# Jisu-Linnea-Han/ClimateMachine.jl

Hardware: AMD Instinct MI355X
Metric: DG RHS DOF-updates/sec (higher is better)
Workload: dtype f64; 1 GPU; Held-Suarez dry GCM (BASELINE configs[2]), stacked cubed sphere 6x30x30x8 elements, N=4, LSRK54 explicit, hyperdiffusion (DryBiharmonic, horizontal), Rusanov, fp64; elements=43200, nodes_per_element=125, states=5, parallelism=element partition (Hilbert, whole columns), 1 rank(s), RCCL p2p halo

## Files before the change

climatemachine.jl_amd/_lib.py:

```python
import ctypes as C
import os

_HERE = os.path.dirname(os.path.abspath(__file__))
LIB_PATH = os.environ.get("CMDG_LIB", os.path.join(_HERE, "libcmdg.so"))

CMDG_K = dict(GRADIENTS=0, DIVGRAD=1, GRADLAP=2, TENDENCY=3, PACK=4, UNPACK=5, UPDATE_AUX=6,
              FILTER=7, STACK_INTEGRAL=8, TRANSPORT=9, HALO_EXPOSED=10, GRADIENTS_EXT=11,
              DIVGRAD_EXT=12, GRADLAP_EXT=13, TENDENCY_EXT=14, FV_GRADIENTS=15, FV_TENDENCY=16,
              ESDG_TENDENCY=17)
STACK_MAXOUT = 8
OPT_KEEP_GRADFLUX = 1
OPT_STACK_HEIGHT = 2
OPT_REFERENCE_HALO = 3
OPT_HALO_PIPELINE = 4
OPT_STEP_GRAPH = 5
OPT_STREAM_PRIORITY = 6
OPT_TENDENCY_PAIRS = 7
OPT_ASYNC_RUN = 8
OPT_TENDENCY_FOUR_WAVES = 9
OPT_GRADARG_HANDOFF = 10
CMDG_Q = dict(GRADFLUX_LIVE=1, LAW_NEEDS_GRADFLUX=2, NDERIVED=3, NUPDATED_AUX=4, FUSED_UPDATE_AUX=5,
              DIRECT_SEND=6, DIRECT_RECV=7, TENDENCY_ELEMS_PER_GROUP=8, HALO_PIPELINE=9, HOST_POST_NS=10, HOST_POST_COUNT=11, GRAPH_STEPS=12, TENDENCY_PAIRS=13,
              GRADARG_HANDOFF=14, GRADARG_REFRESHES=15,
              STATE_READ=16, AUX_READ=20)
# ... 107 lines not shown
    _fields_ = [("volume_flux", C.c_int32), ("surface_flux", C.c_int32), ("Mcut", C.c_double),
                ("low_mach", C.c_int32), ("kinetic_energy_preserving", C.c_int32)]


(ESDG_FLUX_NONE, ESDG_FLUX_ENTROPY_CONSERVATIVE, ESDG_FLUX_CENTRAL, ESDG_FLUX_KG, ESDG_FLUX_RUSANOV,
 ESDG_FLUX_ENTROPY_CONSERVATIVE_PENALTY, ESDG_FLUX_MATRIX) = range(7)
FV_VANLEER, FV_NOLIMITER = 0, 1


_vp, _i32, _i64, _d = C.c_void_p, C.c_int32, C.c_int64, C.c_double
SYMBOLS = [
    ("cmdg_version", C.c_char_p, []),
    ("cmdg_status_string", C.c_char_p, [C.c_int]),
    ("cmdg_physics_counts", C.c_int, [_i32, _vp, _vp]),
    ("cmdg_atmos_host_constants", C.c_int, [_vp, _vp, _vp]),
    ("cmdg_create", C.c_int, [C.POINTER(CmdgDesc), C.POINTER(_vp)]),
    ("cmdg_create_dgfv", C.c_int, [C.POINTER(CmdgDesc), C.POINTER(CmdgFvDesc), C.POINTER(_vp)]),
    ("cmdg_create_esdg", C.c_int, [C.POINTER(CmdgDesc), C.POINTER(CmdgEsdgDesc), C.POINTER(_vp)]),
    ("cmdg_esdg_entropy", C.c_int, [_vp, _vp, _vp, _vp]),
    ("cmdg_destroy", C.c_int, [_vp]),
    ("cmdg_last_error", C.c_char_p, [_vp]),
    ("cmdg_rhs", C.c_int, [_vp, _vp, _vp, _d, _d, _d]),
    ("cmdg_rhs_async", C.c_int, [_vp, _vp, _vp, _d, _d, _d]),
    ("cmdg_lsrk_step", C.c_int, [_vp, _vp, _vp, _d, _d, _i32, _vp, _vp, _vp]),
    ("cmdg_lsrk_run", C.c_int, [_vp, _vp, _vp, _d, _d, _i64, _i32, _vp, _vp, _vp]),
    ("cmdg_synchronize", C.c_int, [_vp]),
    ("cmdg_set_option", C.c_int, [_vp, _i32, _i32]),
    ("cmdg_query", C.c_int, [_vp, _i32, _vp]),
    ("cmdg_export_hypervisc_grad", C.c_int, [_vp, _vp]),
    ("cmdg_export_gradient_flux", C.c_int, [_vp, _vp]),
# ... 108 lines not shown
```

climatemachine.jl_amd/csrc/create.hip:

```cpp
#include <dlfcn.h>

#include <algorithm>
#include <new>

#include "engine_base.h"
#include "laws.h"
#include "reductions.h"

using namespace cmdg;

static thread_local std::string g_create_err;
void cmdg::set_create_err(const std::string &msg) { g_create_err = msg; }

namespace {
struct Law {
    int32_t id;
    EngineBase *(*make)(const cmdg_desc *, std::string &);
    int (*counts)(const int32_t *iparam, int32_t out[6]);
};
const Law LAWS[] = {
    {CMDG_PHYSICS_ADVECTION_DIFFUSION, make_engine_advdiff, counts_advdiff},
    {CMDG_PHYSICS_DRY_ATMOS, make_engine_atmos, counts_atmos},
    {CMDG_PHYSICS_HYDROSTATIC_BOUSSINESQ, make_engine_ocean, counts_ocean},
    {CMDG_PHYSICS_PRESSURE_GRADIENT, make_engine_pgrad, counts_pgrad},
// ... 84 lines not shown
    if (r) g_create_err = err;
    return r;
}

int cmdg_physics_counts(int32_t physics_id, const int32_t *iparam, int32_t out[6])
{
    if (!iparam || !out) return CMDG_ERR_INVALID;
    const Law *law = find_law(physics_id);
    return law ? law->counts(iparam, out) : CMDG_ERR_UNSUPPORTED;
}

int cmdg_atmos_host_constants(const int32_t *iparam, const double *dparam, double out[7])
{
    if (!iparam || !dparam || !out) return CMDG_ERR_INVALID;
    return host_constants_atmos(iparam, dparam, out);
}

static int create_handle(const cmdg_desc *d, const cmdg_fv_desc *fv, cmdg_handle *out, const cmdg_esdg_desc *esdg = nullptr)
{
    *out = nullptr;
    int ndev = 0;
    if (hipGetDeviceCount(&ndev) != hipSuccess || ndev == 0) {
        g_create_err = "no HIP device visible";
        return CMDG_ERR_NO_DEVICE;
    }
    if (d->dim != 3 || d->N[0] != d->N[1]) {
        g_create_err = "only dim == 3 with one horizontal polynomial order is compiled in";
        return CMDG_ERR_UNSUPPORTED;
    }
    if (d->nf_first < CMDG_RUSANOV || d->nf_first > CMDG_ROE_MOIST_LVPP) {
// ... 190 lines not shown
```

climatemachine.jl_amd/csrc/engine.h:

```cpp
#pragma once
#include "engine_base.h"
#include "kernels.h"

namespace cmdg {

template <class P, int NQ_, int NQV_ = NQ_>
struct EngineT : EngineBase {
    typename P::Params prm;
    PassArgs<P> make_args(const RhsCtx &c, const int64_t *elems, int64_t n, int dir, bool exterior, double *send0,
                          double *send1) const
    {
        PassArgs<P> a;
        a.prm = prm;
        a.g = g;
        a.elems = elems;
        a.nelems = n;
        a.Q = c.Qin;
        a.aux = aux;
        a.aux_rw = aux;
        a.derived = derived;
        a.gf = gf;
        a.hypgrad = hypgrad;
        a.hypdiv = hypdiv;
        a.tendency = c.tendency;
// ... 114 lines not shown
        return CMDG_OK;
    }
    bool has_update_aux() const override { return P::HAS_UPDATE_AUX && P::update_aux_active(prm); }
    bool law_needs_gradflux() const override { return P::needs_gradflux(prm); }
    bool gf_node_major() const override { return cmdg::gf_node_major<P>::value; }
    bool fused_update_aux() const override { return P::HAS_UPDATE_AUX && P::FUSE_UPDATE_AUX; }
    bool garg_capable() const override { return HO && !P::needs_gradflux(prm); }
    bool refresh_elidable() const override { return ELIDE; }
    int law_nder() const override { return P::HAS_SOURCE ? P::NDER : 0; }
    int law_nupd() const override { return P::HAS_UPDATE_AUX ? P::NUPD : 0; }
    int tendency_epb() const override { return TendencyShape<P, NQ_, NQV_>::EPB; }
    int law_state_read(int pass) const override { return law_reads<P>::state(pass); }
    int law_aux_read(int pass) const override { return law_reads<P>::aux(pass); }
    int init_derived() override
    {
        if constexpr (P::NDER > 0) {
            const int64_t n = nelem * KDims<NQ_, NQV_>::Np;
            if (derived.alloc((size_t)n * P::NDER) != hipSuccess)
                return fail(CMDG_ERR_HIP, "hipMalloc(derived) failed");
            hipLaunchKernelGGL((k_init_derived<P, NQ_, NQV_>), dim3((unsigned)((n + 255) / 256)), dim3(256),
                               0, s_comp, prm, aux, derived, nelem);
            if (hipStreamSynchronize(s_comp) != hipSuccess)
                return fail(CMDG_ERR_HIP, "k_init_derived failed");
        }
        return CMDG_OK;
    }
};

template <class P, int NQ_, int NQV_ = NQ_>
EngineBase *make_engine(const cmdg_desc *d)
// ... 17 lines not shown
```

climatemachine.jl_amd/csrc/engine_atmos.hip:

```cpp
#include "engine.h"
#include "laws.h"
#include "physics_atmos.h"
#include "with_constant.h"

namespace cmdg {

int counts_atmos(const int32_t *ip, int32_t out[6])
{
    const bool orient = ip[0] != 0, ref = ip[1] != 0, hyp = ip[4] != 0, smag = ip[14] == 1;
    out[0] = 5;
    out[1] = 3 + (orient ? 4 : 0) + (ref ? 7 : 0) + (smag ? 1 : 0) + (hyp ? 1 : 0) + 2;
    out[2] = 4 + (smag ? 1 : 0) + (hyp ? 4 : 0);
    out[3] = 9 + (smag ? 1 : 0);
    out[4] = hyp ? 4 : 0;
    out[5] = hyp ? 12 : 0;
    return CMDG_OK;
}

int host_constants_atmos(const int32_t *ip, const double *dp, double out[7])
{
    static_assert(ATMOS_NHOSTCONST == 7, "cmdg_atmos_host_constants documents seven");
    using P = DryAtmos<false, false, false>;
    P::Params prm;
    P::make_params(prm, ip, dp);
    P::host_constants(prm, out);
    return CMDG_OK;
}

template <int NQ>
static EngineBase *pick(const cmdg_desc *d, std::string &err)
{
    const bool orient = d->iparam[0] != 0, ref = d->iparam[1] != 0, hyp = d->iparam[4] != 0;
    bool mms = (d->iparam[5] & 8) != 0;
    for (int i = 0; i < d->iparam[6] && i < 7; ++i) mms = mms || d->iparam[7 + i] == 2;
    if (mms && (orient || ref || hyp || d->iparam[14] != 0)) {
        err = "DryAtmos: MMSSource / InitStateBC are compiled for NoOrientation, NoReferenceState, "
              "constant viscosity only";
        return nullptr;
    }
    if (d->nf_first >= NF_ROE) {
        if constexpr (NQ == 5) {
// ... 48 lines not shown
```

climatemachine.jl_amd/csrc/kernels.h:

```cpp
#pragma once
#include <type_traits>

#include "cmdg_common.h"

#ifndef CMDG_TEND_MINW
#define CMDG_TEND_MINW 1
#endif
#ifndef CMDG_TEND_EPB_LARGE
#define CMDG_TEND_EPB_LARGE 2
#endif
#ifndef CMDG_TEND_EPB_SMALL
#define CMDG_TEND_EPB_SMALL 1
#endif
#ifndef CMDG_GRAD_MINW
#define CMDG_GRAD_MINW 4
#endif
#ifndef CMDG_GRAD_BOUND_LARGE
#define CMDG_GRAD_BOUND_LARGE 1024
#endif
#ifndef CMDG_LAP_MINW
#define CMDG_LAP_MINW 1
#endif

namespace cmdg {
// ... 69 lines not shown
template <int NQ, int NQV = NQ>
__device__ __forceinline__ void face_setup(const GridDev &g, int64_t e, int t, int f, int n,
                                           FacePt &fp)
{
    int32_t idP;
    int bctag;
    face_index<NQ, NQV>(g, e, t, f, idP, bctag);
    face_geometry<NQ, NQV>(g, e, t, f, n, idP, bctag, fp);
}

template <class P, class = void>
struct has_flux_wavespeed : std::false_type {
};
template <class P>
struct has_flux_wavespeed<P, std::void_t<decltype(P::HAS_FLUX_WAVESPEED)>> : std::true_type {
};

template <class P, class = void>
struct gf_node_major : std::false_type {
};
template <class P>
struct gf_node_major<P, std::void_t<decltype(P::GF_NODE_MAJOR)>>
    : std::integral_constant<bool, P::GF_NODE_MAJOR && (P::NGF > 0)> {
};
template <class P, int Np>
__device__ __forceinline__ int64_t gf_at(int n, int s, int64_t e)
{
    return col_at<gf_node_major<P>::value, P::NGF, Np>(n, s, e);
}
template <class P, int Np>
// ... 254 lines not shown
        const int sidx = surf_index<NQ, NQV>(tid);
#pragma unroll
        for (int s = 0; s < NS; ++s) sQ[s * Np + tid] = lQ[s];
        if (STAGE_M && sidx >= 0) {
#pragma unroll
            for (int s = 0; s < NFA; ++s) sM[s * NSURF + sidx] = laux[P::face_aux(s)];
            if (use_gf) {
#pragma unroll
                for (int s = 0; s < NGF; ++s) sM[(NFA + s) * NSURF + sidx] = lgf[s];
            }
#pragma unroll
            for (int s = 0; s < NHYP; ++s) sM[(NFA + NGFS + s) * NSURF + sidx] = lhyp[s];
        }
        Vec<3 * NS> F, F2;
        F.negzero();
        if constexpr (NCA > 0) {
            Vec<NCA> lc;
            P::node_cache(a.prm, lc, lQ, laux);
            P::flux_first_order_cached(a.prm, F, lQ, laux, lc);
            if (sidx >= 0) {
#pragma unroll
                for (int s = 0; s < NCA; ++s)
                    sM[(OCA + s) * NSURF + sidx] = lc[s];
            }
        } else {
            P::flux_first_order(a.prm, F, lQ, laux, a_t, a.model_dir);
        }
        F2.negzero();
        P::flux_second_order(a.prm, F2, lQ, lgf, lhyp, laux, a_t);
#pragma unroll
        for (int q = 0; q < 3 * NS; ++q) F[q] += F2[q];
        if (hz) {
            if constexpr (!METRICS_FIRST) {
                x11 = vg[XI1X1 * Np], x12 = vg[XI1X2 * Np], x13 = vg[XI1X3 * Np];
                x21 = vg[XI2X1 * Np], x22 = vg[XI2X2 * Np], x23 = vg[XI2X3 * Np];
            }
#pragma unroll
            for (int s = 0; s < NS; ++s) {
                const double F1 = F[3 * s], F2_ = F[3 * s + 1], F3 = F[3 * s + 2];
// ... 1 lines not shown
                sF[(1 * NS + s) * Np + tid] = M * (x21 * F1 + x22 * F2_ + x23 * F3);
            }
        }
        if (vt) {
            if constexpr (!METRICS_FIRST) x31 = vg[XI3X1 * Np], x32 = vg[XI3X2 * Np], x33 = vg[XI3X3 * Np];
#pragma unroll
            for (int s = 0; s < NS; ++s) {
                const double F1 = F[3 * s], F2_ = F[3 * s + 1], F3 = F[3 * s + 2];
                sF[(2 * NS + s) * Np + tid] = M * (x31 * F1 + x32 * F2_ + x33 * F3);
            }
        }
        S.negzero();
        if constexpr (P::HAS_SOURCE) {
            Vec<P::NDER> lder;
            load_state<P::NDER, Np>(lder, a.derived, tid, e);
            P::source(a.prm, S, lQ, lgf, laux, lder, a_t, a.model_dir);
        }
    }
    __syncthreads();
    Vec<NS> Tv;
    if (live && tid < Np) {
        const int i = tid % NQ, j = (tid / NQ) % NQ, k = tid / (NQ * NQ);
        Vec<NS> Tprev;
#pragma unroll
        for (int s = 0; s < NS; ++s) Tprev[s] = 0.0;
        if (a.beta != 0) {
#pragma unroll
            for (int s = 0; s < NS; ++s) Tprev[s] = a.tendency[tid + (int64_t)Np * (s + (int64_t)NS * e)];
        }
        double mDi[NQ], mDj[NQ], mDk[NQV];
#pragma unroll
// ... 786 lines not shown
```

climatemachine.jl_amd/csrc/laws.h:

```cpp
#pragma once
#include <string>

#include "engine_base.h"

namespace cmdg {

EngineBase *make_engine_advdiff(const cmdg_desc *d, std::string &err);
EngineBase *make_engine_advdiff_fv(const cmdg_desc *d, const cmdg_fv_desc *fv, std::string &err);
EngineBase *make_engine_atmos(const cmdg_desc *d, std::string &err);
EngineBase *make_engine_ocean(const cmdg_desc *d, std::string &err);
EngineBase *make_engine_pgrad(const cmdg_desc *d, std::string &err);
EngineBase *make_engine_sw(const cmdg_desc *d, std::string &err);
EngineBase *make_engine_moist(const cmdg_desc *d, std::string &err);
EngineBase *make_engine_se01(const cmdg_desc *d, std::string &err);
EngineBase *make_engine_atmos_linear(const cmdg_desc *d, std::string &err);
EngineBase *make_engine_moist_linear(const cmdg_desc *d, std::string &err);
EngineBase *make_engine_atmos_acoustic(const cmdg_desc *d, std::string &err);
EngineBase *make_engine_esdg(const cmdg_desc *d, const cmdg_esdg_desc *ed, std::string &err);

int counts_advdiff(const int32_t *iparam, int32_t out[6]);
int counts_atmos(const int32_t *iparam, int32_t out[6]);
int counts_ocean(const int32_t *iparam, int32_t out[6]);
int counts_pgrad(const int32_t *iparam, int32_t out[6]);
int counts_sw(const int32_t *iparam, int32_t out[6]);
int counts_moist(const int32_t *iparam, int32_t out[6]);
int counts_ocean_se01(const int32_t *iparam, int32_t out[6]);
int counts_continuity3d_se01(const int32_t *iparam, int32_t out[6]);
int counts_barotropic_se01(const int32_t *iparam, int32_t out[6]);
int counts_atmos_linear(const int32_t *iparam, int32_t out[6]);
int counts_moist_linear(const int32_t *iparam, int32_t out[6]);
int counts_atmos_acoustic(const int32_t *iparam, int32_t out[6]);
int counts_esdg_dryatmos(const int32_t *iparam, int32_t out[6]);
int host_constants_atmos(const int32_t *iparam, const double *dparam, double out[7]);

}
```

climatemachine.jl_amd/csrc/physics_atmos.h:

```cpp
#pragma once
#include "cmdg_common.h"

namespace cmdg {

struct AtmosParams {
    int orient, subtract, kinematic, src, nbc;
    int bc[8];
    double visc, tau, R_d, cp_d, cv_d, T_0, grav, Omega, MSLP, day, invPr, C_smag;
    int withdiv, zero_h;
    double k_a, k_f, k_s;
    double kappa;
    double gamma, gamma_R;
    double R_ratio;
};
static constexpr int ATMOS_NHOSTCONST = 7;

template <bool ORIENT, bool REF, bool HYPER, bool SMAG = false, bool LAWNF = false>
struct DryAtmos {
    static constexpr bool LAW_NF = LAWNF;
    static_assert(!(SMAG && HYPER), "gradient-variable order of this combination is not laid out");
    static_assert(!SMAG || ORIENT, "SmagorinskyLilly needs an orientation (buoyancy correction)");
    using Params = AtmosParams;
    static constexpr int NS = 5;
    static constexpr int OPHI = 3;
    static constexpr int OREF = OPHI + (ORIENT ? 4 : 0);
    static constexpr int OTURB = OREF + (REF ? 7 : 0);
    static constexpr int ODELTA = OTURB + (SMAG ? 1 : 0);
    static constexpr int OMOIST = ODELTA + (HYPER ? 1 : 0);
    static constexpr int NAUX = OMOIST + 2;
    static constexpr int NGRAD = 4 + (SMAG ? 1 : 0) + (HYPER ? 4 : 0);
// ... 50 lines not shown
        p.C_smag = dp[13];
        p.withdiv = ip[15] & 1;
        p.zero_h = (ip[15] >> 1) & 1;
        derive_params(p);
    }
    static void derive_params(Params &p)
    {
        const double day = p.day, R_d = p.R_d, cp_d = p.cp_d, cv_d = p.cv_d;
        p.k_a = 1 / (40 * day);
        p.k_f = 1 / day;
        p.k_s = 1 / (4 * day);
        p.kappa = R_d / cp_d;
        p.gamma = cp_d / cv_d;
        p.gamma_R = p.gamma * R_d;
        p.R_ratio = R_d / R_d;
    }
    static void host_constants(const Params &p, double *out)
    {
        const double c[ATMOS_NHOSTCONST] = {p.k_a, p.k_f, p.k_s, p.kappa, p.gamma, p.gamma_R, p.R_ratio};
        for (int i = 0; i < ATMOS_NHOSTCONST; ++i) out[i] = c[i];
    }

    __device__ static double internal_energy(const Params &, const double *Q, const double *aux)
    {
        const double rho = Q[0];
        const double rhoinv = 1 / rho;
        const double rhoe_kin = rhoinv * (Q[1] * Q[1] + Q[2] * Q[2] + Q[3] * Q[3]) / 2;
        const double e_pot = ORIENT ? aux[OPHI] : -0.0;
        const double rhoe_pot = rho * e_pot;
        const double rhoe_int = Q[4] - rhoe_kin - rhoe_pot;
        return rhoinv * rhoe_int;
    }
    __device__ static double air_T(const Params &m, double e_int) { return m.T_0 + e_int / m.cv_d; }
    __device__ static double air_p(const Params &m, double T, double rho) { return m.R_d * rho * T; }
    __device__ static double soundspeed(const Params &m, double T)
    {
        return sqrt(m.gamma_R * T);
    }

    static constexpr bool MMS_VARIANT = !ORIENT && !REF && !HYPER && !SMAG && !LAWNF;
    static constexpr bool HAS_COURANT = true;
    static constexpr bool HAS_PENALTY = false;
    __device__ static void update_penalty(const Params &, double *, const double *, const double *,
                                          const double *)
    {
    }
    __device__ static double courant(const Params &m, int kind, const double *Q, const double *aux,
                                     const double *gf, double dx, double dt, double, int direction)
// ... 22 lines not shown
            }
            return dt * normnu / (dx * dx);
        }
        const double dotk = Q[1] * k[0] + Q[2] * k[1] + Q[3] * k[2];
        double normu;
        if (direction == DIR_VERTICAL) {
            normu = fabs(dotk) / Q[0];
        } else {
            double v[3];
#pragma unroll
            for (int d = 0; d < 3; ++d)
                v[d] = direction == DIR_HORIZONTAL ? (Q[1 + d] - dotk * k[d]) / Q[0] : Q[1 + d] / Q[0];
            normu = sqrt(v[0] * v[0] + v[1] * v[1] + v[2] * v[2]);
        }
        if (kind == 0) return dt * normu / dx;
        const double ss = soundspeed(m, air_T(m, internal_energy(m, Q, aux)));
        return dt * (normu + ss) / dx;
    }

    __device__ static void flux_first_order(const Params &m, double *F, const double *Q,
                                            const double *aux, double, int)
    {
        const double rho = Q[0];
        const double T = air_T(m, internal_energy(m, Q, aux));
        const double p = air_p(m, T, rho);
        double u[3];
#pragma unroll
        for (int d = 0; d < 3; ++d) u[d] = Q[1 + d] / rho;
#pragma unroll
        for (int d = 0; d < 3; ++d) F[d] = Q[1 + d];
        double pp = p;
        if constexpr (REF) pp = m.subtract ? p - aux[OREF + 1] : p;
#pragma unroll
        for (int c = 0; c < 3; ++c)
#pragma unroll
            for (int d = 0; d < 3; ++d)
                F[d + 3 * (1 + c)] = Q[1 + d] * u[c] + (0.0 + (d == c ? pp : 0.0));
#pragma unroll
        for (int d = 0; d < 3; ++d) F[d + 12] = u[d] * Q[4] + u[d] * p;
    }
    __device__ static double sym(const double *c, int i, int j)
    {
        const int lo = i < j ? i : j, hi = i < j ? j : i;
// ... 72 lines not shown
        }
    }
    __device__ static void init_derived(const Params &, double *der, const double *aux)
    {
        if constexpr (ORIENT) {
            const double phi =
                asin(aux[2] / sqrt(aux[0] * aux[0] + aux[1] * aux[1] + aux[2] * aux[2]));
            der[0] = sin(phi);
            der[1] = cos(phi);
        }
    }
    __device__ static void hs_coeffs(const Params &m, const double *Q, const double *der,
                                     double T, double &k_v, double &k_T, double &T_equil)
    {
        const double k_a = m.k_a, k_f = m.k_f, k_s = m.k_s;
        const double dTy = 60, dthz = 10, T_eq = 315, T_min = 200, sig_b = 7.0 / 10;
        const double p = air_p(m, T, Q[0]);
        const double sig = p / m.MSLP;
        const double exner = pow(sig, m.kappa);
        const double dsig = (sig - sig_b) / (1 - sig_b);
        const double hf = dsig > 0 ? dsig : 0;
        const double s = der[0], c = der[1];
        double Te = (T_eq - dTy * (s * s) - dthz * log(sig) * (c * c)) * exner;
        Te = Te > T_min ? Te : T_min;
        T_equil = Te;
        k_T = k_a + (k_s - k_a) * hf * ((c * c) * (c * c));
        k_v = k_f * hf;
    }
    __device__ static void source(const Params &m, double *S, const double *Q, const double *,
                                  const double *aux, const double *der, double t, int)
    {
        const double rho = Q[0];
        double Sm[3] = {0, 0, 0}, Se = 0;
        bool first = true;
        double T = 0, k_v = 0, k_T = 0, Te = 0;
        if (m.src & 4) {
            T = air_T(m, internal_energy(m, Q, aux));
            hs_coeffs(m, Q, der, T, k_v, k_T, Te);
        }
        if constexpr (ORIENT) {
            if (m.src & 1) {
                double r = rho;
                if constexpr (REF) r = m.subtract ? rho - aux[OREF] : rho;
#pragma unroll
                for (int d = 0; d < 3; ++d) Sm[d] = -r * aux[OPHI + 1 + d];
                first = false;
            }
        }
        if (m.src & 2) {
            const double w = 2 * m.Omega;
            const double c[3] = {-(0 * Q[3] - w * Q[2]), -(w * Q[1] - 0 * Q[3]),
                                 -(0 * Q[2] - 0 * Q[1])};
#pragma unroll
            for (int d = 0; d < 3; ++d) Sm[d] = first ? c[d] : Sm[d] + c[d];
            first = false;
        }
        if constexpr (ORIENT) {
            if (m.src & 4) {
                double k[3];
#pragma unroll
                for (int d = 0; d < 3; ++d) k[d] = aux[OPHI + 1 + d] / m.grav;
                const double kn = k[0] * Q[1] + k[1] * Q[2] + k[2] * Q[3];
#pragma unroll
                for (int d = 0; d < 3; ++d) {
                    const double x = -k_v * (Q[1 + d] - k[d] * kn);
                    Sm[d] = first ? x : Sm[d] + x;
                }
                first = false;
                Se = -k_T * rho * m.cv_d * (T - Te);
            }
        }
        S[0] = 0;
        S[1] = Sm[0];
        S[2] = Sm[1];
        S[3] = Sm[2];
        S[4] = Se;
// ... 88 lines not shown
    }
    __device__ static void gradient_argument(const Params &m, double *G, const double *Q,
                                             const double *aux, double)
    {
        const double rhoinv = 1 / Q[0];
#pragma unroll
        for (int d = 0; d < 3; ++d) G[d] = rhoinv * Q[1 + d];
        const double T = air_T(m, internal_energy(m, Q, aux));
        const double e_tot = Q[4] * (1 / Q[0]);
        G[3] = m.zero_h ? 0.0 : e_tot + m.R_d * T;
        if constexpr (SMAG) G[4] = theta_v(m, T, Q[0]);
        if constexpr (HYPER && ORIENT) {
            double u[3], k[3];
#pragma unroll
            for (int d = 0; d < 3; ++d) u[d] = Q[1 + d] * rhoinv;
#pragma unroll
            for (int d = 0; d < 3; ++d) k[d] = aux[OPHI + 1 + d] / m.grav;
#pragma unroll
            for (int i = 0; i < 3; ++i) {
                double acc = 0;
#pragma unroll
                for (int j = 0; j < 3; ++j) {
                    const double Pij = (i == j ? 1.0 : 0.0) - k[i] * k[j];
                    acc = j == 0 ? Pij * u[j] : acc + Pij * u[j];
                }
                G[4 + i] = acc;
            }
            G[7] = G[3];
        }
    }
    __device__ static double theta_v(const Params &m, double T, double rho)
    {
        const double exner = pow(air_p(m, T, rho) / m.MSLP, m.kappa);
        return m.R_ratio * (T / exner);
    }
    __device__ static void gradient_flux(const Params &m, double *gf, const double *g,
                                         const double *Q, const double *aux, double t)
    {
        double th = 0;
        if constexpr (SMAG) th = theta_v(m, air_T(m, internal_energy(m, Q, aux)), Q[0]);
        gradient_flux_th(m, gf, g, aux, th);
    }
    __device__ static void gradient_flux_g(const Params &m, double *gf, const double *g,
                                           const double *, const double *aux, double,
                                           const double *G)
    {
        gradient_flux_th(m, gf, g, aux, SMAG ? G[SMAG ? 4 : 0] : 0.0);
    }
    __device__ static void gradient_flux_th(const Params &, double *gf, const double *g,
                                            const double *aux, double th)
    {
        if constexpr (SMAG) {
            gf[9] = (g[0 + 3 * 4] * aux[OPHI + 1] + g[1 + 3 * 4] * aux[OPHI + 2] +
                     g[2 + 3 * 4] * aux[OPHI + 3]) / th;
        }
// ... 5 lines not shown
        gf[6] = g[1 + 3 * 1];
        gf[7] = (g[2 + 3 * 1] + g[1 + 3 * 2]) / 2;
        gf[8] = g[2 + 3 * 2];
    }
    __device__ static void post_gradient_laplacian(const Params &m, double *hyp, const double *gl,
                                                   const double *, const double *aux, double)
    {
        if constexpr (HYPER) {
            const double h = aux[ODELTA] / 2;
            const double nu4 = (h * h) * (h * h) / 2 / m.tau;
#pragma unroll
            for (int q = 0; q < 12; ++q) hyp[q] = nu4 * gl[q];
        }
    }
    __device__ static void wavespeed(const Params &m, double *ws, const double *n, const double *Q,
                                     const double *aux, double, int)
    {
        const double rhoinv = 1 / Q[0];
        const double uN =
            fabs(n[0] * (rhoinv * Q[1]) + n[1] * (rhoinv * Q[2]) + n[2] * (rhoinv * Q[3]));
        const double ss = soundspeed(m, air_T(m, internal_energy(m, Q, aux)));
#pragma unroll
        for (int s = 0; s < 5; ++s) ws[s] = uN + ss;
    }
    __device__ static double roe_average(double sM, double sP, double vM, double vP)
    {
        return (sM * vM + sP * vP) / (sM + sP);
    }
    __device__ static void numerical_flux_law(const Params &m, int nf, double *fluxn,
                                              const double *n, const double *QM,
                                              const double *auxM, const double *QP,
                                              const double *auxP, double t, int facedir)
    {
        double FM[15], FP[15];
#pragma unroll
        for (int i = 0; i < 15; ++i) FM[i] = FP[i] = -0.0;
        flux_first_order(m, FM, QM, auxM, t, facedir);
        flux_first_order(m, FP, QP, auxP, t, facedir);
        const double rM = QM[0], rP = QP[0];
        double uM[3], uP[3];
#pragma unroll
        for (int d = 0; d < 3; ++d) {
            uM[d] = QM[1 + d] / rM;
            uP[d] = QP[1 + d] / rP;
        }
        const double TM = air_T(m, internal_energy(m, QM, auxM));
        const double TP = air_T(m, internal_energy(m, QP, auxP));
        const double pM = air_p(m, TM, rM), pP = air_p(m, TP, rP);
        const double cM = soundspeed(m, TM), cP = soundspeed(m, TP);
        const double unM = uM[0] * n[0] + uM[1] * n[1] + uM[2] * n[2];
        const double unP = uP[0] * n[0] + uP[1] * n[1] + uP[2] * n[2];
        if (nf == NF_LMARS) {
            double ppM = pM, ppP = pP;
            if constexpr (REF)
                if (m.subtract) {
                    ppM -= auxM[OREF + 1];
                    ppP -= auxP[OREF + 1];
                }
            const double hM = m.zero_h ? 0.0 : QM[4] / rM + m.R_d * TM;
            const double hP = m.zero_h ? 0.0 : QP[4] / rP + m.R_d * TP;
            const double beta = 1.0;
            const double u_half = 1.0 / 2 * (unP + unM) - beta * 1 / (rM + rP) / cM * (ppP - ppM);
// ... 70 lines not shown
        } else if (0 <= SP) {
#pragma unroll
            for (int s = 0; s < 5; ++s)
                fluxn[s] += (S0 * (SP * QP[s] - fnP[s]) + SP * pD[s]) / (SP - S0);
        } else {
#pragma unroll
            for (int s = 0; s < 5; ++s) fluxn[s] += fnP[s];
        }
    }
    __device__ static void update_aux(const Params &m, const double *Q, double *aux, double)
    {
        static_assert(!GRADARG_REFRESH_UNREAD ||
                          (upd_aux(0) == NAUX - NUPD && aux_read(0) <= NAUX - NUPD &&
                           aux_read(2) <= NAUX - NUPD && aux_read(3) <= NAUX - NUPD),
                      "a pass that reads moisture.theta_v / air_T needs the refresh in every update");
        const double T = air_T(m, internal_energy(m, Q, aux));
        aux[OMOIST] = theta_v(m, T, Q[0]);
        aux[OMOIST + 1] = T;
    }
    __device__ static void boundary_state(const Params &m, int kind, int bctag, double *QP,
                                          double *auxP, const double *n, const double *QM,
                                          const double *, double t, const double *, const double *)
    {
        if constexpr (MMS_VARIANT) {
            if (m.bc[bctag - 1] == 2) {
                mms_state(t, auxP[0], auxP[1], auxP[2], QP);
                return;
            }
        }
        if (m.bc[bctag - 1] == 1) {
            const double dn = QM[1] * n[0] + QM[2] * n[1] + QM[3] * n[2];
// ... 39 lines not shown
```

include/cmdg.h:

```cpp
#ifndef CMDG_H
#define CMDG_H
#include <stdint.h>

#ifdef __cplusplus
extern "C" {
#endif

typedef struct cmdg_context *cmdg_handle;

typedef enum cmdg_status {
    CMDG_OK = 0,
    CMDG_ERR_INVALID = -1,
    CMDG_ERR_HIP = -2,
    CMDG_ERR_NO_DEVICE = -3,
    CMDG_ERR_COMM = -4,
    CMDG_ERR_UNSUPPORTED = -5
} cmdg_status;

enum { CMDG_EVERY_DIRECTION = 0, CMDG_HORIZONTAL_DIRECTION = 1, CMDG_VERTICAL_DIRECTION = 2 };
enum {
    CMDG_RUSANOV = 0, CMDG_CENTRAL_FIRST_ORDER = 1,
    CMDG_ROE = 2, CMDG_HLLC = 3, CMDG_LMARS = 4,
    CMDG_ROE_MOIST = 5, CMDG_ROE_MOIST_LM = 6, CMDG_ROE_MOIST_HH = 7, CMDG_ROE_MOIST_LV = 8,
    CMDG_ROE_MOIST_LVPP = 9
// ... 39 lines not shown
    int32_t nnabr;
    const int32_t *nabrtorank;
    const int64_t *nabrtovmapsend;
    const int64_t *nabrtovmaprecv;
    double *state_auxiliary;
    double *state_gradient_flux;
    double *Qhypervisc_grad;
    double *Qhypervisc_div;
    const double *Dv;
} cmdg_desc;

const char *cmdg_version(void);
const char *cmdg_status_string(int status);
int cmdg_physics_counts(int32_t physics_id, const int32_t *iparam, int32_t out[6]);
int cmdg_atmos_host_constants(const int32_t *iparam, const double *dparam, double out[7]);

int cmdg_create(const cmdg_desc *desc, cmdg_handle *out);
int cmdg_destroy(cmdg_handle h);

enum { CMDG_FV_CONSTANT = 0, CMDG_FV_LINEAR = 1 };
enum { CMDG_FV_VANLEER = 0, CMDG_FV_NOLIMITER = 1 };
typedef struct cmdg_fv_desc {
    int32_t reconstruction;
    int32_t width;
    int32_t limiter;
    int32_t nvertelem;
    int32_t periodicstack;
} cmdg_fv_desc;
int cmdg_create_dgfv(const cmdg_desc *desc, const cmdg_fv_desc *fv, cmdg_handle *out);

// ... 323 lines not shown
```

Before: 19.81 billion DOF-updates/s.

## Replace fp64 divisions with refined reciprocals and share per-node thermodynamics

Divisions by uniform physical constants (cv_d, grav, MSLP, Held-Suarez sigma denominator) and by density are replaced with multiplication by a Newton-refined reciprocal plus a div_fixup correction. A wave-wide ballot falls back to true division when any operand's exponent is outside a safe window. Reciprocals of the constants are precomputed on the device at engine init. In the volume tendency kernel, velocity, 1/rho and temperature are computed once per node through a NodeThermo struct and reused by flux_first_order and source. The goal is to cut expensive fp64 division sequences and duplicated thermodynamic work, at the cost of extra code paths and a host-device round trip at init.

```diff
diff --git a/climatemachine.jl_amd/_lib.py b/climatemachine.jl_amd/_lib.py
--- a/climatemachine.jl_amd/_lib.py
+++ b/climatemachine.jl_amd/_lib.py
@@ -145,6 +145,7 @@
     ("cmdg_status_string", C.c_char_p, [C.c_int]),
     ("cmdg_physics_counts", C.c_int, [_i32, _vp, _vp]),
     ("cmdg_atmos_host_constants", C.c_int, [_vp, _vp, _vp]),
+    ("cmdg_atmos_fdiv_constants", C.c_int, [_vp, _vp, _vp, _vp, _vp, _i32, _vp]),
     ("cmdg_create", C.c_int, [C.POINTER(CmdgDesc), C.POINTER(_vp)]),
     ("cmdg_create_dgfv", C.c_int, [C.POINTER(CmdgDesc), C.POINTER(CmdgFvDesc), C.POINTER(_vp)]),
     ("cmdg_create_esdg", C.c_int, [C.POINTER(CmdgDesc), C.POINTER(CmdgEsdgDesc), C.POINTER(_vp)]),
diff --git a/climatemachine.jl_amd/csrc/create.hip b/climatemachine.jl_amd/csrc/create.hip
--- a/climatemachine.jl_amd/csrc/create.hip
+++ b/climatemachine.jl_amd/csrc/create.hip
@@ -122,6 +122,15 @@
 {
     if (!iparam || !dparam || !out) return CMDG_ERR_INVALID;
     return host_constants_atmos(iparam, dparam, out);
+}
+
+int cmdg_atmos_fdiv_constants(const int32_t *iparam, const double *dparam, double rcp[4], int32_t *ok,
+                              const double *num, int32_t nnum, double *quot)
+{
+    if (!iparam || !dparam || !rcp || !ok || nnum < 0 || (nnum > 0 && (!num || !quot))) return CMDG_ERR_INVALID;
+    int ndev = 0;
+    if (hipGetDeviceCount(&ndev) != hipSuccess || ndev == 0) return CMDG_ERR_NO_DEVICE;
+    return fdiv_constants_atmos(iparam, dparam, rcp, ok, num, nnum, quot);
 }
 
 static int create_handle(const cmdg_desc *d, const cmdg_fv_desc *fv, cmdg_handle *out, const cmdg_esdg_desc *esdg = nullptr)
diff --git a/climatemachine.jl_amd/csrc/engine.h b/climatemachine.jl_amd/csrc/engine.h
--- a/climatemachine.jl_amd/csrc/engine.h
+++ b/climatemachine.jl_amd/csrc/engine.h
@@ -3,6 +3,13 @@
 #include "kernels.h"
 
 namespace cmdg {
+
+template <class P, class = void>
+struct has_device_params : std::false_type {
+};
+template <class P>
+struct has_device_params<P, std::void_t<decltype(&P::device_params)>> : std::true_type {
+};
 
 template <class P, int NQ_, int NQV_ = NQ_>
 struct EngineT : EngineBase {
@@ -152,6 +159,10 @@
     int law_aux_read(int pass) const override { return law_reads<P>::aux(pass); }
     int init_derived() override
     {
+        if constexpr (has_device_params<P>::value) {
+            if (P::device_params(prm, s_comp) != hipSuccess)
+                return fail(CMDG_ERR_HIP, "device_params failed");
+        }
         if constexpr (P::NDER > 0) {
             const int64_t n = nelem * KDims<NQ_, NQV_>::Np;
             if (derived.alloc((size_t)n * P::NDER) != hipSuccess)
diff --git a/climatemachine.jl_amd/csrc/engine_atmos.hip b/climatemachine.jl_amd/csrc/engine_atmos.hip
--- a/climatemachine.jl_amd/csrc/engine_atmos.hip
+++ b/climatemachine.jl_amd/csrc/engine_atmos.hip
@@ -25,6 +25,39 @@
     P::make_params(prm, ip, dp);
     P::host_constants(prm, out);
     return CMDG_OK;
+}
+
+static __global__ void k_atmos_div_uniform(AtmosParams prm, const double *num, int nnum, double *quot)
+{
+    using P = DryAtmos<false, false, false>;
+    const int t = blockIdx.x * blockDim.x + threadIdx.x;
+    if (t >= nnum) return;
+    double d[ATMOS_NRCP];
+    P::uniform_divisors(prm, d);
+#pragma unroll
+    for (int i = 0; i < ATMOS_NRCP; ++i) quot[(int64_t)i * nnum + t] = P::div_uniform(prm, i, d[i], num[t]);
+}
+int fdiv_constants_atmos(const int32_t *ip, const double *dp, double *out_rcp, int32_t *out_ok, const double *num,
+                         int32_t nnum, double *quot)
+{
+    using P = DryAtmos<false, false, false>;
+    P::Params prm;
+    P::make_params(prm, ip, dp);
+    if (P::device_params(prm, nullptr) != hipSuccess) return CMDG_ERR_HIP;
+    for (int i = 0; i < ATMOS_NRCP; ++i) out_rcp[i] = prm.rcp[i];
+    *out_ok = prm.fdiv_ok;
+    if (nnum <= 0) return CMDG_OK;
+    double *dev = nullptr;
+    if (hipMalloc(&dev, sizeof(double) * nnum * (1 + ATMOS_NRCP)) != hipSuccess) return CMDG_ERR_HIP;
+    hipError_t r = hipMemcpy(dev, num, sizeof(double) * nnum, hipMemcpyHostToDevice);
+    if (r == hipSuccess) {
+        hipLaunchKernelGGL(k_atmos_div_uniform, dim3((unsigned)((nnum + 255) / 256)), dim3(256), 0, nullptr, prm, dev,
+                           (int)nnum, dev + nnum);
+        r = hipGetLastError();
+    }
+    if (r == hipSuccess) r = hipMemcpy(quot, dev + nnum, sizeof(double) * nnum * ATMOS_NRCP, hipMemcpyDeviceToHost);
+    (void)hipFree(dev);
+    return r == hipSuccess ? CMDG_OK : CMDG_ERR_HIP;
 }
 
 template <int NQ>
diff --git a/climatemachine.jl_amd/csrc/fdiv.h b/climatemachine.jl_amd/csrc/fdiv.h
--- /dev/null
+++ b/climatemachine.jl_amd/csrc/fdiv.h
@@ -0,0 +1,55 @@
+#pragma once
+#include <hip/hip_runtime.h>
+
+namespace cmdg {
+
+static constexpr int FDIV_WINDOW = 256;
+
+__device__ __forceinline__ int fdiv_exp(double x) { return __builtin_amdgcn_frexp_exp(x); }
+__device__ __forceinline__ bool fdiv_exp_in_window(int e)
+{
+    return (unsigned)(e + FDIV_WINDOW) < 2u * FDIV_WINDOW;
+}
+__device__ __forceinline__ bool fdiv_in_window(double x) { return fdiv_exp_in_window(fdiv_exp(x)); }
+__device__ __forceinline__ bool fdiv_in_window3(double a, double b, double c)
+{
+    const int ea = fdiv_exp(a), eb = fdiv_exp(b), ec = fdiv_exp(c);
+    const int lo = min(min(ea, eb), ec), hi = max(max(ea, eb), ec);
+    return lo >= -FDIV_WINDOW && hi < FDIV_WINDOW;
+}
+__device__ __forceinline__ bool fdiv_in_window_nonzero(double x)
+{
+    return fabs(x) >= 0x1p-256 && fabs(x) <= 0x1p254;
+}
+__device__ __forceinline__ bool fdiv_wave_all(bool ok) { return __builtin_amdgcn_ballot_w64(!ok) == 0; }
+
+__device__ __forceinline__ double fdiv_refined_rcp(double d)
+{
+    const double y0 = __builtin_amdgcn_rcp(d);
+    const double e0 = __builtin_fma(-d, y0, 1.0);
+    const double y1 = __builtin_fma(y0, e0, y0);
+    const double e1 = __builtin_fma(-d, y1, 1.0);
+    return __builtin_fma(y1, e1, y1);
+}
+
+struct SharedDivisor {
+    double d, y;
+    __device__ __forceinline__ explicit SharedDivisor(double d_) : d(d_), y(fdiv_refined_rcp(d_)) {}
+    __device__ __forceinline__ SharedDivisor(double d_, double y_) : d(d_), y(y_) {}
+    __device__ __forceinline__ double div_in_window(double n) const
+    {
+        const double q0 = n * y;
+        const double r = __builtin_fma(-d, q0, n);
+        return __builtin_amdgcn_div_fixup(__builtin_fma(r, y, q0), d, n);
+    }
+    __device__ __forceinline__ double div(double n) const
+    {
+        return fdiv_in_window(n) && fdiv_in_window(d) ? div_in_window(n) : n / d;
+    }
+    __device__ __forceinline__ double div_wave(double n, bool d_ok) const
+    {
+        return d_ok && fdiv_wave_all(fdiv_in_window(n)) ? div_in_window(n) : n / d;
+    }
+};
+
+}
diff --git a/climatemachine.jl_amd/csrc/kernels.h b/climatemachine.jl_amd/csrc/kernels.h
--- a/climatemachine.jl_amd/csrc/kernels.h
+++ b/climatemachine.jl_amd/csrc/kernels.h
@@ -107,6 +107,22 @@
 };
 template <class P>
 struct has_flux_wavespeed<P, std::void_t<decltype(P::HAS_FLUX_WAVESPEED)>> : std::true_type {
+};
+
+template <class P, class = void>
+struct has_node_thermo : std::false_type {
+};
+template <class P>
+struct has_node_thermo<P, std::void_t<decltype(P::HAS_NODE_THERMO)>> : std::true_type {
+};
+template <class P, bool = has_node_thermo<P>::value>
+struct node_thermo_of {
+    struct type {
+    };
+};
+template <class P>
+struct node_thermo_of<P, true> {
+    using type = typename P::NodeThermo;
 };
 
 template <class P, class = void>
@@ -391,6 +407,7 @@
         }
         Vec<3 * NS> F, F2;
         F.negzero();
+        [[maybe_unused]] typename node_thermo_of<P>::type lth;
         if constexpr (NCA > 0) {
             Vec<NCA> lc;
             P::node_cache(a.prm, lc, lQ, laux);
@@ -400,6 +417,9 @@
                 for (int s = 0; s < NCA; ++s)
                     sM[(OCA + s) * NSURF + sidx] = lc[s];
             }
+        } else if constexpr (has_node_thermo<P>::value) {
+            P::node_thermo(a.prm, lth, lQ, laux);
+            P::flux_first_order(a.prm, lth, F, lQ, laux, a_t, a.model_dir);
         } else {
             P::flux_first_order(a.prm, F, lQ, laux, a_t, a.model_dir);
         }
@@ -431,7 +451,10 @@
         if constexpr (P::HAS_SOURCE) {
             Vec<P::NDER> lder;
             load_state<P::NDER, Np>(lder, a.derived, tid, e);
-            P::source(a.prm, S, lQ, lgf, laux, lder, a_t, a.model_dir);
+            if constexpr (has_node_thermo<P>::value && NCA == 0)
+                P::source(a.prm, lth, S, lQ, lgf, laux, lder, a_t, a.model_dir);
+            else
+                P::source(a.prm, S, lQ, lgf, laux, lder, a_t, a.model_dir);
         }
     }
     __syncthreads();
diff --git a/climatemachine.jl_amd/csrc/laws.h b/climatemachine.jl_amd/csrc/laws.h
--- a/climatemachine.jl_amd/csrc/laws.h
+++ b/climatemachine.jl_amd/csrc/laws.h
@@ -32,5 +32,7 @@
 int counts_atmos_acoustic(const int32_t *iparam, int32_t out[6]);
 int counts_esdg_dryatmos(const int32_t *iparam, int32_t out[6]);
 int host_constants_atmos(const int32_t *iparam, const double *dparam, double out[7]);
+int fdiv_constants_atmos(const int32_t *iparam, const double *dparam, double *out_rcp, int32_t *out_ok,
+                         const double *num, int32_t nnum, double *quot);
 
 }
diff --git a/climatemachine.jl_amd/csrc/physics_atmos.h b/climatemachine.jl_amd/csrc/physics_atmos.h
--- a/climatemachine.jl_amd/csrc/physics_atmos.h
+++ b/climatemachine.jl_amd/csrc/physics_atmos.h
@@ -1,5 +1,8 @@
 #pragma once
+#include <cmath>
+
 #include "cmdg_common.h"
+#include "fdiv.h"
 
 namespace cmdg {
 
@@ -12,8 +15,18 @@
     double kappa;
     double gamma, gamma_R;
     double R_ratio;
+    double rcp[4];
+    int fdiv_ok;
 };
 static constexpr int ATMOS_NHOSTCONST = 7;
+static constexpr int ATMOS_NRCP = 4;
+enum { ATMOS_DIV_CV_D = 0, ATMOS_DIV_GRAV = 1, ATMOS_DIV_MSLP = 2, ATMOS_DIV_HS_SIGMA = 3 };
+static constexpr double ATMOS_HS_SIGMA_B = 7.0 / 10;
+
+static __global__ void k_atmos_reciprocals(const double *d, double *y)
+{
+    if (threadIdx.x < ATMOS_NRCP) y[threadIdx.x] = fdiv_refined_rcp(d[threadIdx.x]);
+}
 
 template <bool ORIENT, bool REF, bool HYPER, bool SMAG = false, bool LAWNF = false>
 struct DryAtmos {
@@ -94,6 +107,42 @@
         p.gamma = cp_d / cv_d;
         p.gamma_R = p.gamma * R_d;
         p.R_ratio = R_d / R_d;
+        for (int i = 0; i < ATMOS_NRCP; ++i) p.rcp[i] = 0;
+        p.fdiv_ok = 0;
+    }
+    __host__ __device__ static void uniform_divisors(const Params &p, double *d)
+    {
+        d[ATMOS_DIV_CV_D] = p.cv_d;
+        d[ATMOS_DIV_GRAV] = p.grav;
+        d[ATMOS_DIV_MSLP] = p.MSLP;
+        d[ATMOS_DIV_HS_SIGMA] = 1 - ATMOS_HS_SIGMA_B;
+    }
+    static hipError_t device_params(Params &p, hipStream_t st)
+    {
+        double h[2 * ATMOS_NRCP], *dev = nullptr;
+        uniform_divisors(p, h);
+        hipError_t r = hipMalloc(&dev, sizeof(h));
+        if (r != hipSuccess) return r;
+        r = hipMemcpyAsync(dev, h, sizeof(double) * ATMOS_NRCP, hipMemcpyHostToDevice, st);
+        if (r == hipSuccess) {
+            hipLaunchKernelGGL(k_atmos_reciprocals, dim3(1), dim3(64), 0, st, dev, dev + ATMOS_NRCP);
+            r = hipGetLastError();
+        }
+        if (r == hipSuccess)
+            r = hipMemcpyAsync(h + ATMOS_NRCP, dev + ATMOS_NRCP, sizeof(double) * ATMOS_NRCP, hipMemcpyDeviceToHost, st);
+        if (r == hipSuccess) r = hipStreamSynchronize(st);
+        (void)hipFree(dev);
+        if (r != hipSuccess) return r;
+        p.fdiv_ok = 0;
+        for (int i = 0; i < ATMOS_NRCP; ++i) {
+            int e = 0;
+            const double d = h[i];
+            std::frexp(d, &e);
+            const bool ok = d != 0 && std::isfinite(d) && e >= -FDIV_WINDOW && e < FDIV_WINDOW;
+            p.rcp[i] = ok ? h[ATMOS_NRCP + i] : 0.0;
+            if (ok) p.fdiv_ok |= 1 << i;
+        }
+        return hipSuccess;
     }
     static void host_constants(const Params &p, double *out)
     {
@@ -101,17 +150,84 @@
         for (int i = 0; i < ATMOS_NHOSTCONST; ++i) out[i] = c[i];
     }
 
-    __device__ static double internal_energy(const Params &, const double *Q, const double *aux)
-    {
+    __device__ static double div_uniform(const Params &m, int i, double d, double n)
+    {
+        if constexpr (SMAG) return n / d;
+        const SharedDivisor s(d, m.rcp[i]);
+        double q = s.div_in_window(n);
+        if (__builtin_expect(!(((m.fdiv_ok >> i) & 1) && fdiv_wave_all(fdiv_in_window_nonzero(n))), 0)) {
+            __asm__ volatile("");
+            q = n / d;
+        }
+        return q;
+    }
+    __device__ static void vertical_unit(const Params &m, const double *aux, double *k)
+    {
+        if constexpr (SMAG) {
+#pragma unroll
+            for (int d = 0; d < 3; ++d) k[d] = aux[OPHI + 1 + d] / m.grav;
+            return;
+        }
+        const SharedDivisor s(m.grav, m.rcp[ATMOS_DIV_GRAV]);
+#pragma unroll
+        for (int d = 0; d < 3; ++d) k[d] = s.div_in_window(aux[OPHI + 1 + d]);
+        const bool ok = fdiv_in_window3(aux[OPHI + 1], aux[OPHI + 2], aux[OPHI + 3]);
+        if (__builtin_expect(!(((m.fdiv_ok >> ATMOS_DIV_GRAV) & 1) && fdiv_wave_all(ok)), 0)) {
+            __asm__ volatile("");
+#pragma unroll
+            for (int d = 0; d < 3; ++d) k[d] = aux[OPHI + 1 + d] / m.grav;
+        }
+    }
+    struct NodeThermo {
+        double rhoinv, u[3], T;
+    };
+    static constexpr bool HAS_NODE_THERMO = true;
+    __device__ static void node_thermo(const Params &m, NodeThermo &th, const double *Q, const double *aux)
+    {
+        if constexpr (SMAG) {
+            node_thermo_plain(m, th, Q, aux);
+            return;
+        }
         const double rho = Q[0];
-        const double rhoinv = 1 / rho;
+        const SharedDivisor s(rho);
+        th.rhoinv = s.div_in_window(1.0);
+#pragma unroll
+        for (int d = 0; d < 3; ++d) th.u[d] = s.div_in_window(Q[1 + d]);
+        const bool ok = fdiv_in_window(rho) && fdiv_in_window3(Q[1], Q[2], Q[3]);
+        if (__builtin_expect(!fdiv_wave_all(ok), 0)) {
+            __asm__ volatile("");
+            th.rhoinv = 1 / rho;
+#pragma unroll
+            for (int d = 0; d < 3; ++d) th.u[d] = Q[1 + d] / rho;
+        }
+        th.T = air_T(m, internal_energy(m, Q, aux, th.rhoinv));
+    }
+    __device__ static void node_thermo_plain(const Params &m, NodeThermo &th, const double *Q, const double *aux)
+    {
+        const double rho = Q[0];
+        th.rhoinv = 1 / rho;
+#pragma unroll
+        for (int d = 0; d < 3; ++d) th.u[d] = Q[1 + d] / rho;
+        th.T = air_T_plain(m, internal_energy(m, Q, aux, th.rhoinv));
+    }
+    __device__ static double air_T_plain(const Params &m, double e_int) { return m.T_0 + e_int / m.cv_d; }
+    __device__ static double internal_energy(const Params &m, const double *Q, const double *aux)
+    {
+        return internal_energy(m, Q, aux, 1 / Q[0]);
+    }
+    __device__ static double internal_energy(const Params &, const double *Q, const double *aux, double rhoinv)
+    {
+        const double rho = Q[0];
         const double rhoe_kin = rhoinv * (Q[1] * Q[1] + Q[2] * Q[2] + Q[3] * Q[3]) / 2;
         const double e_pot = ORIENT ? aux[OPHI] : -0.0;
         const double rhoe_pot = rho * e_pot;
         const double rhoe_int = Q[4] - rhoe_kin - rhoe_pot;
         return rhoinv * rhoe_int;
     }
-    __device__ static double air_T(const Params &m, double e_int) { return m.T_0 + e_int / m.cv_d; }
+    __device__ static double air_T(const Params &m, double e_int)
+    {
+        return m.T_0 + div_uniform(m, ATMOS_DIV_CV_D, m.cv_d, e_int);
+    }
     __device__ static double air_p(const Params &m, double T, double rho) { return m.R_d * rho * T; }
     __device__ static double soundspeed(const Params &m, double T)
     {
@@ -164,19 +280,24 @@
             normu = sqrt(v[0] * v[0] + v[1] * v[1] + v[2] * v[2]);
         }
         if (kind == 0) return dt * normu / dx;
-        const double ss = soundspeed(m, air_T(m, internal_energy(m, Q, aux)));
+        const double ss = soundspeed(m, air_T_plain(m, internal_energy(m, Q, aux)));
         return dt * (normu + ss) / dx;
     }
 
     __device__ static void flux_first_order(const Params &m, double *F, const double *Q,
+                                            const double *aux, double t, int dir)
+    {
+        NodeThermo th;
+        node_thermo_plain(m, th, Q, aux);
+        flux_first_order(m, th, F, Q, aux, t, dir);
+    }
+    __device__ static void flux_first_order(const Params &m, const NodeThermo &th, double *F, const double *Q,
                                             const double *aux, double, int)
     {
         const double rho = Q[0];
-        const double T = air_T(m, internal_energy(m, Q, aux));
+        const double T = th.T;
         const double p = air_p(m, T, rho);
-        double u[3];
-#pragma unroll
-        for (int d = 0; d < 3; ++d) u[d] = Q[1 + d] / rho;
+        const double *u = th.u;
 #pragma unroll
         for (int d = 0; d < 3; ++d) F[d] = Q[1 + d];
         double pp = p;
@@ -279,11 +400,11 @@
                                      double T, double &k_v, double &k_T, double &T_equil)
     {
         const double k_a = m.k_a, k_f = m.k_f, k_s = m.k_s;
-        const double dTy = 60, dthz = 10, T_eq = 315, T_min = 200, sig_b = 7.0 / 10;
+        const double dTy = 60, dthz = 10, T_eq = 315, T_min = 200, sig_b = ATMOS_HS_SIGMA_B;
         const double p = air_p(m, T, Q[0]);
-        const double sig = p / m.MSLP;
+        const double sig = div_uniform(m, ATMOS_DIV_MSLP, m.MSLP, p);
         const double exner = pow(sig, m.kappa);
-        const double dsig = (sig - sig_b) / (1 - sig_b);
+        const double dsig = div_uniform(m, ATMOS_DIV_HS_SIGMA, 1 - sig_b, sig - sig_b);
         const double hf = dsig > 0 ? dsig : 0;
         const double s = der[0], c = der[1];
         double Te = (T_eq - dTy * (s * s) - dthz * log(sig) * (c * c)) * exner;
@@ -292,15 +413,23 @@
         k_T = k_a + (k_s - k_a) * hf * ((c * c) * (c * c));
         k_v = k_f * hf;
     }
-    __device__ static void source(const Params &m, double *S, const double *Q, const double *,
-                                  const double *aux, const double *der, double t, int)
+    __device__ static void source(const Params &m, double *S, const double *Q, const double *gf,
+                                  const double *aux, const double *der, double t, int dir)
+    {
+        NodeThermo th;
+        th.T = 0;
+        if (m.src & 4) node_thermo_plain(m, th, Q, aux);
+        source(m, th, S, Q, gf, aux, der, t, dir);
+    }
+    __device__ static void source(const Params &m, const NodeThermo &th, double *S, const double *Q,
+                                  const double *, const double *aux, const double *der, double t, int)
     {
         const double rho = Q[0];
         double Sm[3] = {0, 0, 0}, Se = 0;
         bool first = true;
         double T = 0, k_v = 0, k_T = 0, Te = 0;
         if (m.src & 4) {
-            T = air_T(m, internal_energy(m, Q, aux));
+            T = th.T;
             hs_coeffs(m, Q, der, T, k_v, k_T, Te);
         }
         if constexpr (ORIENT) {
@@ -323,8 +452,7 @@
         if constexpr (ORIENT) {
             if (m.src & 4) {
                 double k[3];
-#pragma unroll
-                for (int d = 0; d < 3; ++d) k[d] = aux[OPHI + 1 + d] / m.grav;
+                vertical_unit(m, aux, k);
                 const double kn = k[0] * Q[1] + k[1] * Q[2] + k[2] * Q[3];
 #pragma unroll
                 for (int d = 0; d < 3; ++d) {
@@ -443,8 +571,7 @@
             double u[3], k[3];
 #pragma unroll
             for (int d = 0; d < 3; ++d) u[d] = Q[1 + d] * rhoinv;
-#pragma unroll
-            for (int d = 0; d < 3; ++d) k[d] = aux[OPHI + 1 + d] / m.grav;
+            vertical_unit(m, aux, k);
 #pragma unroll
             for (int i = 0; i < 3; ++i) {
                 double acc = 0;
@@ -467,7 +594,7 @@
                                          const double *Q, const double *aux, double t)
     {
         double th = 0;
-        if constexpr (SMAG) th = theta_v(m, air_T(m, internal_energy(m, Q, aux)), Q[0]);
+        if constexpr (SMAG) th = theta_v(m, air_T_plain(m, internal_energy(m, Q, aux)), Q[0]);
         gradient_flux_th(m, gf, g, aux, th);
     }
     __device__ static void gradient_flux_g(const Params &m, double *gf, const double *g,
@@ -503,12 +630,19 @@
         }
     }
     __device__ static void wavespeed(const Params &m, double *ws, const double *n, const double *Q,
-                                     const double *aux, double, int)
-    {
-        const double rhoinv = 1 / Q[0];
+                                     const double *aux, double t, int dir)
+    {
+        NodeThermo th;
+        node_thermo_plain(m, th, Q, aux);
+        wavespeed(m, th, ws, n, Q, aux, t, dir);
+    }
+    __device__ static void wavespeed(const Params &m, const NodeThermo &th, double *ws, const double *n,
+                                     const double *Q, const double *, double, int)
+    {
+        const double rhoinv = th.rhoinv;
         const double uN =
             fabs(n[0] * (rhoinv * Q[1]) + n[1] * (rhoinv * Q[2]) + n[2] * (rhoinv * Q[3]));
-        const double ss = soundspeed(m, air_T(m, internal_energy(m, Q, aux)));
+        const double ss = soundspeed(m, th.T);
 #pragma unroll
         for (int s = 0; s < 5; ++s) ws[s] = uN + ss;
     }
@@ -524,17 +658,14 @@
         double FM[15], FP[15];
 #pragma unroll
         for (int i = 0; i < 15; ++i) FM[i] = FP[i] = -0.0;
-        flux_first_order(m, FM, QM, auxM, t, facedir);
-        flux_first_order(m, FP, QP, auxP, t, facedir);
+        NodeThermo thM, thP;
+        node_thermo_plain(m, thM, QM, auxM);
+        node_thermo_plain(m, thP, QP, auxP);
+        flux_first_order(m, thM, FM, QM, auxM, t, facedir);
+        flux_first_order(m, thP, FP, QP, auxP, t, facedir);
         const double rM = QM[0], rP = QP[0];
-        double uM[3], uP[3];
-#pragma unroll
-        for (int d = 0; d < 3; ++d) {
-            uM[d] = QM[1 + d] / rM;
-            uP[d] = QP[1 + d] / rP;
-        }
-        const double TM = air_T(m, internal_energy(m, QM, auxM));
-        const double TP = air_T(m, internal_energy(m, QP, auxP));
+        const double *uM = thM.u, *uP = thP.u;
+        const double TM = thM.T, TP = thP.T;
         const double pM = air_p(m, TM, rM), pP = air_p(m, TP, rP);
         const double cM = soundspeed(m, TM), cP = soundspeed(m, TP);
         const double unM = uM[0] * n[0] + uM[1] * n[1] + uM[2] * n[2];
@@ -635,7 +766,7 @@
                           (upd_aux(0) == NAUX - NUPD && aux_read(0) <= NAUX - NUPD &&
                            aux_read(2) <= NAUX - NUPD && aux_read(3) <= NAUX - NUPD),
                       "a pass that reads moisture.theta_v / air_T needs the refresh in every update");
-        const double T = air_T(m, internal_energy(m, Q, aux));
+        const double T = air_T_plain(m, internal_energy(m, Q, aux));
         aux[OMOIST] = theta_v(m, T, Q[0]);
         aux[OMOIST + 1] = T;
     }
diff --git a/include/cmdg.h b/include/cmdg.h
--- a/include/cmdg.h
+++ b/include/cmdg.h
@@ -77,6 +77,8 @@
 const char *cmdg_status_string(int status);
 int cmdg_physics_counts(int32_t physics_id, const int32_t *iparam, int32_t out[6]);
 int cmdg_atmos_host_constants(const int32_t *iparam, const double *dparam, double out[7]);
+int cmdg_atmos_fdiv_constants(const int32_t *iparam, const double *dparam, double rcp[4], int32_t *ok,
+                              const double *num, int32_t nnum, double *quot);
 
 int cmdg_create(const cmdg_desc *desc, cmdg_handle *out);
 int cmdg_destroy(cmdg_handle h);
```

After: 19.78 billion DOF-updates/s. No clear change (-0.1%).
